# LesleyLai/cuda-path-tracer

Measured on AMD Instinct MI355X. Metric: Mrays/s at 1920×1080, 8 bounces, higher is better.
Workload: dtype f32

## Files before the change

cuda-path-tracer_amd/csrc/pt_bvh_gpu.hip:

```cpp
#include <hip/hip_runtime.h>

#include <algorithm>
#include <vector>

#include "../../include/ptcore.h"
#include "pt_bvh_rules.hpp"
#include "pt_device.hpp"
#include "pt_layout_rules.hpp"

namespace pt {
using namespace bvh_rules;
namespace {

constexpr uint32_t kFinished = 0xffffffffu;
constexpr uint32_t kBinWords = kBuckets * 7u;
constexpr uint32_t kSerialNode = 32u;

__device__ __forceinline__ uint32_t enc(float f)
{
  const uint32_t b = __float_as_uint(f);
  return (b & 0x80000000u) ? ~b : (b | 0x80000000u);
}
__device__ __forceinline__ float dec(uint32_t e) { return __uint_as_float((e & 0x80000000u) ? (e & 0x7fffffffu) : ~e); }

// ... 695 lines not shown
  layout_rules::quantise_node(q, nk, lo, hi, refs);
  uint4* out = reinterpret_cast<uint4*>(w.nodes_q) + 4u * (size_t)w.wbegin[x];
  for (int j = 0; j < 4; ++j) out[j] = make_uint4(q[4 * j], q[4 * j + 1], q[4 * j + 2], q[4 * j + 3]);
}

__global__ __launch_bounds__(256) void k_lay_instance_tris(m4 m, const float* positions, const uint32_t* indices,
                                                           const uint32_t* tri_order, uint32_t T, float4* out)
{
  const uint32_t k = blockIdx.x * 256u + threadIdx.x;
  if (k >= T) return;
  const uint32_t* idx = indices + 3u * (size_t)tri_order[k];
  const float* q0 = positions + 3u * (size_t)idx[0];
  const float* q1 = positions + 3u * (size_t)idx[1];
  const float* q2 = positions + 3u * (size_t)idx[2];
  layout_rules::instance_triangle(m, mk3(q0[0], q0[1], q0[2]), mk3(q1[0], q1[1], q1[2]), mk3(q2[0], q2[1], q2[2]), out + kTriVec4 * (size_t)k);
}

}

int build_layouts_device(hipStream_t stream, const float4* d_bvh, uint32_t count, const std::vector<uint32_t>& level_base,
                         DeviceLayouts* out)
{
  *out = DeviceLayouts{};
  if (count == 0u) return PTC_OK;
  if (level_base.size() < 2u || level_base.front() != 0u || level_base.back() != count) return PTC_ERR_INVALID;
  const uint32_t T = (count + 1u) / 2u;
  const size_t N = count;
  Pool pool;
  LayoutWork w{};
  w.tree.bvh = d_bvh;
// ... 59 lines not shown
  out->dummy_ref = w.dummy_ref;
  out->root_min[0] = root[0].x; out->root_min[1] = root[0].y; out->root_min[2] = root[0].z;
  out->root_max[0] = root[1].x; out->root_max[1] = root[1].y; out->root_max[2] = root[1].z;
  outputs.allocs.clear();
  return PTC_OK;
}

void launch_instance_triangles(hipStream_t stream, const m4& m, const float* d_positions, const uint32_t* d_indices,
                               const uint32_t* d_tri_order, uint32_t triangles, float4* d_out)
{
  if (triangles == 0u) return;
  hipLaunchKernelGGL(k_lay_instance_tris, dim3((triangles + 255u) / 256u), dim3(256), 0, stream, m, d_positions, d_indices,
                     d_tri_order, triangles, d_out);
}

}
```

cuda-path-tracer_amd/csrc/pt_device.hpp:

```cpp
#pragma once

#include <hip/hip_runtime.h>
#include <stdint.h>

#include <vector>

#include "../../include/ptcore.h"
#include "pt_math.hpp"

namespace pt {

constexpr int kWave = 64;
constexpr int kChunk = 64;
constexpr int kStackDepth = 64;
constexpr int kMaxBounces = 64;
constexpr int kWorkSlots = 4;
#ifndef PT_T4_LDS
#define PT_T4_LDS 24
#endif
constexpr int kLds4 = PT_T4_LDS;
static_assert(kLds4 >= 4 && kLds4 <= kStackDepth, "PT_T4_LDS out of range");

constexpr uint32_t kFlagStackOverflow = 1u;
constexpr uint32_t kFlagDispatchOrder = 2u;
// ... 17 lines not shown

#ifndef PT_TRI_VEC4
#define PT_TRI_VEC4 4
#endif
constexpr uint32_t kTriVec4 = PT_TRI_VEC4;
constexpr uint32_t kLeafBit = 0x80000000u;
constexpr uint32_t kNoChild = 0xffffffffu;

struct DMeshView {
  const float* positions;
  const uint32_t* indices;
  const float4* bvh;
  const float4* wide;
  const float4* leaf_parent;
  const uint4* bvh4q;
  uint32_t bvh4_root;
  uint32_t dummy_ref;
  float root_min[3];
  float root_max[3];
  uint32_t root_ref;
  uint32_t bvh_node_count;
};

struct DBand {
  uint32_t pix_begin, width, rank, nranks, block_rows;
};
PT_HD uint32_t band_pixel(const DBand& b, uint32_t s)
{
  if (b.nranks <= 1u) return b.pix_begin + s;
  const uint32_t lr = s / b.width, x = s - lr * b.width;
// ... 16 lines not shown
  uint32_t width;
  DBand band;
  uint8_t beam_of[32];
};
constexpr uint32_t kSphereTab = 8u;
struct DScene {
  const DObject* objects;
  const uint32_t* object_material;
  const float4* spheres;
  const DMaterial* materials;
  DMeshView cur;
  const DMeshView* mesh_views;
  const uint32_t* object_mesh;
  const float4* tris;
  const uint32_t* object_tri_base;
  uint32_t* slow_stack;
  uint2* spill;
  uint32_t spill_stride;
  uint32_t spill_cap;
  uint32_t lds_cap;
  uint32_t force_slow;
  uint32_t static_eighths;
  uint32_t refill_lanes;
  uint32_t split_idle;
  uint32_t object_count;
  const float4* sphere_ball;
  uint32_t lanes_run;
  uint32_t fold_run;
  DBeam beam;
};
// ... 104 lines not shown
                     std::vector<uint32_t>* level_base);

struct DeviceLayouts {
  uint32_t* nodes_q = nullptr;
  float4* leaf_parent = nullptr;
  uint32_t* tri_order = nullptr;
  float4* wide = nullptr;
  uint32_t wide4_nodes = 0, wide4_depth = 0, triangles = 0, inner_nodes = 0;
  uint32_t root_ref4 = 0, root_ref2 = 0, dummy_ref = 0;
  float root_min[3] = {0, 0, 0}, root_max[3] = {0, 0, 0};
};
int build_layouts_device(hipStream_t stream, const float4* d_bvh, uint32_t count, const std::vector<uint32_t>& level_base,
                         DeviceLayouts* out);
void launch_instance_triangles(hipStream_t stream, const m4& m, const float* d_positions, const uint32_t* d_indices,
                               const uint32_t* d_tri_order, uint32_t triangles, float4* d_out);

void launch_raygen(hipStream_t s, const DCameras& cams, const DBatchInfo& bi, DBand band, uint32_t pix_count,
                   DPaths paths, DeviceCounters* counters, const DObject* objects = nullptr, uint32_t filt_begin = 0u,
                   uint32_t filt_end = 0u, uint32_t* worklist = nullptr, DHits hits = DHits{nullptr, nullptr},
                   unsigned long long* tile_desc = nullptr, uint32_t tile_stride = 0u, uint32_t epoch = 0u,
                   bool finish_misses = false, DFrame fb = DFrame{nullptr, nullptr}, bool staged = false);
void launch_trace(hipStream_t s, const DScene& scene, DPaths paths, DHits hits, uint32_t max_paths, int bounce,
                  DeviceCounters* counters, bool count_tests, int variant);
void launch_spheres(hipStream_t s, const DScene& scene, uint32_t obj_begin, uint32_t obj_end, bool first, DPaths paths, DHits hits,
                    uint32_t max_paths, int bounce, DeviceCounters* counters, const DBatchInfo& bi, uint32_t filt_begin = 0u,
                    uint32_t filt_end = 0u, uint32_t* worklist = nullptr, unsigned long long* tile_desc = nullptr,
                    uint32_t tile_stride = 0u, uint32_t epoch = 0u);
void launch_traverse_run(hipStream_t s, const DScene& scene, uint32_t obj_begin, uint32_t obj_end, bool first, DPaths paths,
                         DHits hits, int bounce, int work_slot, DeviceCounters* counters, bool count_tests, uint32_t waves,
                         uint32_t* slow_list, const uint32_t* order, const DBatchInfo& bi, bool listed = false);
// ... 55 lines not shown
```

cuda-path-tracer_amd/csrc/pt_kernels.hip:

```cpp




#include "pt_device.hpp"
#include "pt_rng.hpp"
#include "pt_beam_rules.hpp"
#include "pt_feed_rules.hpp"
static_assert(pt::beam_rules::kLeaf == pt::kLeafBit, "pt_beam_rules.hpp restates the leaf bit of the four-wide node (pt_device.hpp)");
static_assert((uint32_t)pt::beam_rules::kEntries == pt::kBeamEntries, "pt_beam_rules.hpp restates the entries per tile (pt_device.hpp)");
static_assert(pt::feed_rules::kBatch == (uint32_t)pt::kWave, "a feed batch is one wavefront's worth of rays");
#include <float.h>

namespace pt {

#include "pt_kernels_common.inc"

template <bool kCount>
__global__ __launch_bounds__(kWave) void k_trace(DScene sc, DPaths paths, DHits hits, int bounce, DeviceCounters* counters)
{
  __shared__ uint32_t s_stack[kStackDepth * kWave];
  const uint32_t n = counters->live[bounce];
  const uint32_t s = blockIdx.x * kWave + threadIdx.x;
  if (blockIdx.x * kWave >= n) return;
  bool hit = false;
// ... 74 lines not shown
  generate_ray(cam, x0, y1, o, d01);
  generate_ray(cam, x1, y1, o, d11);
  generate_ray(cam, 0.5f * (x0 + x1), 0.5f * (y0 + y1), o, dc);
  const beam_rules::Frustum fr = beam_rules::make_frustum(xform_point(obj->inv_m, o), xform_vector(obj->inv_m, d00), xform_vector(obj->inv_m, d10),
                                                          xform_vector(obj->inv_m, d01), xform_vector(obj->inv_m, d11), xform_vector(obj->inv_m, dc));
  f3 lo4[4], hi4[4];
  uint32_t ref4[4];
  int n = 0;
  if (sc.cur.bvh_node_count != 0u)
    n = beam_rules::tile_entries(reinterpret_cast<const uint32_t*>(sc.cur.bvh4q), node_count4, sc.cur.bvh4_root, ld3(sc.cur.root_min), ld3(sc.cur.root_max), fr,
                                 lo4, hi4, ref4);
  float4* e = out + (size_t)id * (2u * kBeamEntries);
#pragma unroll
  for (int k = 0; k < (int)kBeamEntries; ++k) {
    if (k < n) {
      e[2 * k] = make_float4(lo4[k].x, lo4[k].y, lo4[k].z, __uint_as_float(ref4[k]));
      e[2 * k + 1] = make_float4(hi4[k].x, hi4[k].y, hi4[k].z, 0.0f);
    } else {
      e[2 * k] = make_float4(__builtin_inff(), __builtin_inff(), __builtin_inff(), __uint_as_float(kNoChild));
      e[2 * k + 1] = make_float4(-__builtin_inff(), -__builtin_inff(), -__builtin_inff(), 0.0f);
    }
  }
}

template <bool kCount, bool kFirst, bool kBeam = false>
__global__ __launch_bounds__(kWave) __attribute__((amdgpu_waves_per_eu(PT_T4_WAVES, PT_T4_WAVES)))
void k_traverse4(DScene sc, uint32_t obj_index, DPaths paths, DHits hits, int bounce, int work_slot,
                 DeviceCounters* counters, uint32_t* slow_list, const uint32_t* order, DBatchInfo bi, int listed)
{
  traverse4_walk<kCount, kFirst, kBeam>(sc, obj_index, paths, hits, bounce, work_slot, counters, slow_list, order, bi, listed != 0);
  uint32_t prev = 0u;
// ... 150 lines not shown
```

cuda-path-tracer_amd/csrc/pt_layout_rules.hpp:

```cpp
#pragma once

#include <cmath>

#include "pt_math.hpp"

namespace pt {
namespace layout_rules {

PT_HD void collapse_costs(float area_x, const float* bl, const float* br, float* b)
{
  float node_cost = bl[0] + br[2];
  node_cost = sel_min(node_cost, bl[1] + br[1]);
  node_cost = sel_min(node_cost, bl[2] + br[0]);
  b[0] = area_x + node_cost;
  b[1] = sel_min(b[0], bl[0] + br[0]);
  b[2] = sel_min(b[1], sel_min(bl[0] + br[1], bl[1] + br[0]));
  b[3] = sel_min(b[2], node_cost);
}

template <class Tree>
PT_HD int choose_children(const Tree& tree, const float* best, uint32_t x, uint32_t kids[4])
{
  int nk = 0;
  uint32_t stack_x[4];
// ... 63 lines not shown
        q[4 + a] = lo_q;
        q[7 + a] = hi_q;
        break;
      }
      ++e;
    }
    q[a] = __builtin_bit_cast(uint32_t, origin);
    exps |= (uint32_t)(e + 127) << (8 * a);
  }
  q[3] = (exps & 0xffu) << 23;
  q[10] = ((exps >> 8) & 0xffu) << 23;
  q[11] = ((exps >> 16) & 0xffu) << 23;
  for (int k = 0; k < 4; ++k) q[12 + k] = refs[k];
}

PT_HD void instance_triangle(const m4& m, f3 q0, f3 q1, f3 q2, float4* out)
{
  const f3 p0 = xform_point(m, q0), p1 = xform_point(m, q1), p2 = xform_point(m, q2);
  const f3 e1 = p1 - p0;
  const f3 e2 = p2 - p0;
  const f3 n = normalize(cross(e1, e2));
  out[0] = make_float4(p0.x, p0.y, p0.z, e1.x);
  out[1] = make_float4(e1.y, e1.z, e2.x, e2.y);
  out[2] = make_float4(e2.z, n.x, n.y, n.z);
}

}
}
```

cuda-path-tracer_amd/csrc/pt_walk.inc:

```
struct BatchFeed {
  DeviceCounters* ctr;
  uint32_t stride, count, bounce, work_slot, static_eighths, dyn_batch;
  bool listed;
  __device__ __forceinline__ uint32_t rays_of(uint32_t f) const { return listed ? ctr[f].list_count : ctr[f].live[bounce]; }
  uint32_t home_f, home_r, home_base, home_rs, stat_next, stat_step, stat_count;
  bool in_static, done;

  static __device__ __forceinline__ uint32_t region_size_of(uint32_t n) { return feed_rules::region_size_of(n); }
  static __device__ __forceinline__ uint32_t region_len_of(uint32_t n, uint32_t rs, uint32_t r) { return feed_rules::region_len_of(n, rs, r); }
  static __device__ __forceinline__ uint32_t pos_of(uint32_t rs, uint32_t r, uint32_t local) { return feed_rules::pos_of(rs, r, local); }
  __device__ __forceinline__ uint32_t static_batches_of(uint32_t len) const
  {
    return feed_rules::static_batches_of(len, static_eighths);
  }
  __device__ __forceinline__ void init(DeviceCounters* ctr_, const DBatchInfo& bi, int bounce_, int work_slot_,
                                       uint32_t static_eighths_, bool listed_ = false)
  {
    ctr = ctr_;
    listed = listed_;
    stride = bi.stride;
    count = bi.count;
    bounce = (uint32_t)bounce_;
    work_slot = (uint32_t)work_slot_;
    static_eighths = gridDim.x >= 8u * count ? static_eighths_ : 0u;
// ... 283 lines not shown
  __shared__ unsigned long long s_grp_best[kWave];
  __shared__ uint32_t s_grp_count[kWave];
  __shared__ uint32_t s_leader[kWave];
  __shared__ uint32_t s_pair[kWave];
  typedef __attribute__((address_space(3))) uint32_t lds_u32;
  lds_u32* stack = (lds_u32*)s_stack + threadIdx.x;
  const uint32_t gid = blockIdx.x * kWave + threadIdx.x;
  uint32_t n_max = 0u;
  if (!kPersist) {
    for (uint32_t f = 0; f < bi.count; ++f) n_max = max(n_max, listed ? counters[f].list_count : counters[f].live[bounce]);
    if (n_max == 0u) return 0;
  }
  const DObject* obj = sc.objects + obj_index;
  const uint32_t mat = sc.object_material[obj_index];
  const float4* tris = sc.tris + kTriVec4 * (size_t)sc.object_tri_base[obj_index];
  if (!kPersist && blockIdx.x >= ((n_max + kWave - 1u) / kWave + 8u) * bi.count) return 0;
  auto uni = [](float v) { return __uint_as_float((uint32_t)__builtin_amdgcn_readfirstlane((int)__float_as_uint(v))); };
  const f3 obj_bmin = mk3(uni(obj->bmin[0]), uni(obj->bmin[1]), uni(obj->bmin[2]));
  const f3 obj_bmax = mk3(uni(obj->bmax[0]), uni(obj->bmax[1]), uni(obj->bmax[2]));
#ifdef PT_TAILPROF
  const unsigned long long tp_start = wall_clock64();
  unsigned long long tp_exhausted = 0ull;
  uint32_t tp_iters = 0u, tp_splits = 0u, tp_iters_exh = 0u, tp_lanes_exh = 0u;
  unsigned long long tp_c_split = 0ull, tp_c_retire = 0ull, tp_c_step = 0ull, tp_lanes_tail = 0ull;
#endif
  BatchFeed feed;
  PersistFeed pfeed;
  if (kPersist) {
    pfeed.init(pa->st, counters, bi, blockIdx.x);
    if (threadIdx.x < (uint32_t)kMaxBatch) s_pend[threadIdx.x] = 0u;
// ... 166 lines not shown
      limit = d_limit;
      slot = d_slot;
      cur = ((lds_u32*)s_stack)[d_sbase * kWave + (int)d];
      sp = sbase = 0;
      ray_boxes = 0u;
      const uint32_t leader = s_leader[d];
      s_leader[threadIdx.x] = leader;
      __hip_atomic_fetch_add(&s_grp_count[leader], 1u, __ATOMIC_RELAXED, __HIP_MEMORY_SCOPE_WORKGROUP);
      active = true;
    }
    if (can_give && drank < pairs) ++sbase;
  };

  auto step = [&]() {
    if (active) {
      const bool is_leaf = (cur & kLeafBit) != 0u;
      const uint32_t index = cur & ~kLeafBit;
      typedef uint32_t u32x4 __attribute__((ext_vector_type(4)));
      u32x4 w0, w1, w2, w3;
      constexpr bool kLeaf48 = kTriVec4 == 3u;
      const char* rec = is_leaf ? reinterpret_cast<const char*>(tris) + (16u * kTriVec4) * (size_t)index
                                : reinterpret_cast<const char*>(sc.cur.bvh4q) + 64u * (size_t)index;
      const char* rec3 = rec + (kLeaf48 && is_leaf ? 32 : 48);
      const int top = sp - 1;
      const uint32_t below_addr = (uint32_t)(uintptr_t)(stack + min(max(top, 0), lds_cap - 1) * kWave);
      uint32_t below;
      asm volatile(
          "global_load_dwordx4 %0, %5, off\n\t"
          "global_load_dwordx4 %1, %5, off offset:16\n\t"
          "global_load_dwordx4 %2, %5, off offset:32\n\t"
          "global_load_dwordx4 %3, %6, off\n\t"
          "ds_read_b32 %4, %7\n\t"
          "s_waitcnt vmcnt(0) lgkmcnt(0)"
          : "=&v"(w0), "=&v"(w1), "=&v"(w2), "=&v"(w3), "=&v"(below)
          : "v"(rec), "v"(rec3), "v"(below_addr)
          : "memory");
      if (__builtin_expect(top >= lds_cap, 0)) below = sc.spill[(size_t)(top - lds_cap) * sc.spill_stride + gid].x;
      below = top >= sbase ? below : kNoChild;
      const uint4 q0 = make_uint4(w0.x, w0.y, w0.z, w0.w), q1 = make_uint4(w1.x, w1.y, w1.z, w1.w);
      const uint4 q2 = make_uint4(w2.x, w2.y, w2.z, w2.w), q3 = make_uint4(w3.x, w3.y, w3.z, w3.w);
      if (!is_leaf) {
        if (kCount) ++tally.nodes;
        const f3 org = mk3(__uint_as_float(q0.x), __uint_as_float(q0.y), __uint_as_float(q0.z));
        const f3 ax = mk3(__uint_as_float(q0.w) * inv.x, __uint_as_float(q2.z) * inv.y, __uint_as_float(q2.w) * inv.z);
        const f3 bn = mk3(__builtin_fmaf(org.x, inv.x, oin.x), __builtin_fmaf(org.y, inv.y, oin.y), __builtin_fmaf(org.z, inv.z, oin.z));
        const f3 bf = mk3(__builtin_fmaf(org.x, inv.x, oif.x), __builtin_fmaf(org.y, inv.y, oif.y), __builtin_fmaf(org.z, inv.z, oif.z));
        const uint32_t nqx = neg_x ? q1.w : q1.x, fqx = neg_x ? q1.x : q1.w;
        const uint32_t nqy = neg_y ? q2.x : q1.y, fqy = neg_y ? q1.y : q2.x;
        const uint32_t nqz = neg_z ? q2.y : q1.z, fqz = neg_z ? q1.z : q2.y;
        float key[4];
        uint32_t ref[4] = {q3.x, q3.y, q3.z, q3.w};
#pragma unroll
        for (int c = 0; c < 4; ++c) {
          const float cnx = (float)((nqx >> (8 * c)) & 0xffu), cny = (float)((nqy >> (8 * c)) & 0xffu), cnz = (float)((nqz >> (8 * c)) & 0xffu);
          const float cfx = (float)((fqx >> (8 * c)) & 0xffu), cfy = (float)((fqy >> (8 * c)) & 0xffu), cfz = (float)((fqz >> (8 * c)) & 0xffu);
          const float tn = fmaxf(fmaxf(fmaxf(__builtin_fmaf(cnx, ax.x, bn.x), __builtin_fmaf(cny, ax.y, bn.y)),
                                       __builtin_fmaf(cnz, ax.z, bn.z)), 0.0f);
          const float tf = fminf(fminf(fminf(__builtin_fmaf(cfx, ax.x, bf.x), __builtin_fmaf(cfy, ax.y, bf.y)),
                                       __builtin_fmaf(cfz, ax.z, bf.z)), limit);
          if (kCount && ref[c] != sc.cur.dummy_ref) { ++tally.boxes; ++ray_boxes; }
          key[c] = tn <= tf ? tn : __builtin_inff();
        }
        auto cx = [&](int a, int b) {
          const bool sw = key[b] < key[a];
          const float ka = sw ? key[b] : key[a], kb = sw ? key[a] : key[b];
          const uint32_t ra = sw ? ref[b] : ref[a], rb = sw ? ref[a] : ref[b];
          key[a] = ka;
          key[b] = kb;
          ref[a] = ra;
          ref[b] = rb;
        };
        cx(0, 1);
        cx(2, 3);
        cx(0, 2);
        cx(1, 3);
// ... 8 lines not shown
          stack[sp * kWave] = ref[1];
          sp += key[1] < __builtin_inff() ? 1 : 0;
        } else {
          if (key[3] < __builtin_inff()) push(ref[3]);
          if (key[2] < __builtin_inff()) push(ref[2]);
          if (key[1] < __builtin_inff()) push(ref[1]);
        }
        if (key[0] < __builtin_inff()) {
          cur = ref[0];
        } else {
          cur = below;
          sp = max(sp - 1, sbase);
        }
      } else {
        if (kCount) ++tally.tris;
        const f3 p0 = mk3(__uint_as_float(q0.x), __uint_as_float(q0.y), __uint_as_float(q0.z));
        const f3 e1 = mk3(__uint_as_float(q0.w), __uint_as_float(q1.x), __uint_as_float(q1.y));
        const f3 e2 = mk3(__uint_as_float(q1.z), __uint_as_float(q1.w), __uint_as_float(q2.x));
#if PT_FLAT_TRI
        const f3 h = cross(rd, e2);
        const float a = dot(e1, h);
        const f3 sv = ro - p0;
        const float f = 1.0f / a;
        const float u = f * dot(sv, h);
        const f3 qv = cross(sv, e1);
        const float w = f * dot(rd, qv);
        const float t = f * dot(e2, qv);
        const bool hit = !(a > -0.0000001f && a < 0.0000001f) & !(u < 0.0f || u > 1.0f) & !(w < 0.0f || u + w > 1.0f) &
                         !(t < tmin) & (t < best_t || (t == best_t && (int)index > best_k));
        best_t = hit ? t : best_t;
// ... 105 lines not shown
          if (__builtin_expect(!(finite_f(inv.x) && finite_f(inv.y) && finite_f(inv.z) && finite_f(tol.x + tol.y + tol.z)) ||
                               sc.force_slow == 1u, 0)) {
            if (kPersist) set_aside(counters + cur_frame, pa->slow_list + (size_t)cur_frame * bi.stride, slot & kSlotMask);
            else set_aside(counters, slow_list, slot);
            wrote = true;
            go = false;
          } else {
            oin = oi - tol;
            oif = oi + tol;
            neg_x = inv.x < 0.0f;
            neg_y = inv.y < 0.0f;
            neg_z = inv.z < 0.0f;
            best_t = t_in;
            best_k = -1;
            limit = scale * best_t * 1.001f;
            cur = sc.cur.bvh4_root;
            sp = sbase = 0;
            ray_boxes = 0u;
            if (kBeam) {
              float key[4];
              uint32_t ref[4];
#pragma unroll
              for (int c = 0; c < 4; ++c) {
                const float4 lo = eb[2 * c], hi = eb[2 * c + 1];
                const float tn = fmaxf(fmaxf(fmaxf(__builtin_fmaf(neg_x ? hi.x : lo.x, inv.x, oin.x), __builtin_fmaf(neg_y ? hi.y : lo.y, inv.y, oin.y)),
                                             __builtin_fmaf(neg_z ? hi.z : lo.z, inv.z, oin.z)), 0.0f);
                const float tf = fminf(fminf(fminf(__builtin_fmaf(neg_x ? lo.x : hi.x, inv.x, oif.x), __builtin_fmaf(neg_y ? lo.y : hi.y, inv.y, oif.y)),
                                             __builtin_fmaf(neg_z ? lo.z : hi.z, inv.z, oif.z)), limit);
                key[c] = tn <= tf ? tn : __builtin_inff();
                ref[c] = __float_as_uint(lo.w);
                if (kCount && key[c] < __builtin_inff()) { ++tally.boxes; ++ray_boxes; }
// ... 133 lines not shown
```

cuda-path-tracer_amd/csrc/ptcore_checks.cpp:

```cpp
#include "ptcore_ctx.hpp"

using namespace pt;
using namespace ptcd;

extern "C" {

int ptc_check_beam(const float* positions, uint32_t vertex_count, const uint32_t* indices, uint32_t index_count, const float* object_m16,
                   const ptc_camera* camera, uint32_t width, uint32_t height, uint32_t stride, uint64_t* stats5, float* entries_out)
{
  if (!positions || !indices || !camera || index_count == 0u || index_count % 3u || width < 2u || height < 2u || stride == 0u) return PTC_ERR_INVALID;
  std::vector<ptc_bvh_node> nodes((size_t)index_count / 3u * 2u);
  uint32_t depth = 0;
  const int rc = build_bvh(positions, vertex_count, indices, index_count, nodes.data(), &depth);
  if (rc < 0) return rc;
  WideAccel wide;
  if (int r = build_wide(nodes.data(), (uint32_t)rc, wide)) return r;
  Wide4Accel w4;
  if (int r = build_wide4(nodes.data(), (uint32_t)rc, w4)) return r;
  m4 m{};
  for (int c = 0; c < 4; ++c)
    for (int r = 0; r < 4; ++r) m.c[c][r] = object_m16 ? object_m16[4 * c + r] : (c == r ? 1.0f : 0.0f);
  const m4 inv_m = inverse(m);
  const DCamera cam = make_camera(*camera, width, height);
  auto gen = [&](float fx, float fy, f3& o, f3& d) {
// ... 51 lines not shown
      }
      if (ref >= n4) return HitRec{true, 0xffffffffu, -1.0f};
      const uint32_t* q = nq + 16u * (size_t)ref;
      for (int c = 0; c < 4; ++c) {
        f3 lo, hi;
        if (!beam_rules::child_box(q, c, lo, hi)) continue;
        if (slab(lo, hi, o, inv, best.t)) stack.push_back(q[12 + c]);
      }
    }
    return best;
  };
  uint64_t tiles = 0, empty = 0, entries = 0, rays = 0, hits = 0;
  int bad = 0;
  const uint32_t tiles_x = (width + kBeamTile - 1u) / kBeamTile, tiles_y = (height + kBeamTile - 1u) / kBeamTile;
  const uint32_t root_ref4[1] = {w4.root_ref};
  for (uint32_t ty = 0; ty < tiles_y; ++ty)
    for (uint32_t tx = 0; tx < tiles_x; ++tx) {
      const float x0 = (float)(tx * kBeamTile) - 0.05f, x1 = (float)((tx + 1u) * kBeamTile) + 0.05f;
      const float y0 = (float)(ty * kBeamTile) - 0.05f, y1 = (float)((ty + 1u) * kBeamTile) + 0.05f;
      f3 o, d00, d10, d01, d11, dc;
      gen(x0, y0, o, d00);
      gen(x1, y0, o, d10);
      gen(x0, y1, o, d01);
      gen(x1, y1, o, d11);
      gen(0.5f * (x0 + x1), 0.5f * (y0 + y1), o, dc);
      const beam_rules::Frustum fr = beam_rules::make_frustum(xform_point(inv_m, o), xform_vector(inv_m, d00), xform_vector(inv_m, d10),
                                                              xform_vector(inv_m, d01), xform_vector(inv_m, d11), xform_vector(inv_m, dc));
      f3 lo4[4], hi4[4];
      uint32_t ref4[4];
      const int n = beam_rules::tile_entries(nq, n4, w4.root_ref, root_lo, root_hi, fr, lo4, hi4, ref4);
      if (entries_out) {
        float* e = entries_out + ((size_t)ty * tiles_x + tx) * 32u;
        for (int k = 0; k < 4; ++k) {
          const float inf = __builtin_inff();
          uint32_t ref = k < n ? ref4[k] : kNoChild;
          float refbits;
          std::memcpy(&refbits, &ref, 4);
          const float rec[8] = {k < n ? lo4[k].x : inf, k < n ? lo4[k].y : inf, k < n ? lo4[k].z : inf, refbits,
                                k < n ? hi4[k].x : -inf, k < n ? hi4[k].y : -inf, k < n ? hi4[k].z : -inf, 0.0f};
          std::memcpy(e + 8 * k, rec, sizeof rec);
        }
      }
      ++tiles;
      empty += n == 0;
      entries += (uint64_t)n;
      for (int k = 0; k < n; ++k)
        if (!(ref4[k] & kLeafBit) && ref4[k] >= n4) ++bad;
      for (uint32_t py = ty * kBeamTile; py < std::min(height, (ty + 1u) * kBeamTile); py += stride)
        for (uint32_t px = tx * kBeamTile; px < std::min(width, (tx + 1u) * kBeamTile); px += stride) {
          const float jit[5][2] = {{0.0f, 0.0f}, {1.0f, 0.0f}, {0.0f, 1.0f}, {1.0f, 1.0f}, {0.5f, 0.5f}};
// ... 240 lines not shown
```

cuda-path-tracer_amd/csrc/ptcore_ctx.hpp:

```cpp
#pragma once

#include "../../include/ptcore.h"

#include <hip/hip_runtime.h>

#include <algorithm>
#include <chrono>
#include <cmath>
#include <cstddef>
#include <cstdio>
#include <cstdlib>
#include <cstring>
#include <new>
#include <string>
#include <unordered_map>
#include <vector>

#include "pt_device.hpp"
#include "pt_host.hpp"
#include "pt_beam_rules.hpp"
#include "pt_feed_rules.hpp"

using namespace pt;

// ... 130 lines not shown
  bool sphere_lanes = true;
  bool sphere_fold = true;
  bool beam = true;
  int persist = 0;
  uint32_t persist_service_every = 5;
  uint32_t persist_help_tiles = 8;
  uint32_t persist_min_frames = 2;
  uint64_t scene_serial = 0;
  uint32_t beam_tiles_x = 0, beam_tiles_y = 0;
  uint32_t traverse_waves = 5120;
  uint32_t refill_lanes = 32;
  uint32_t static_eighths = 4;
  bool merge_instances = true;
  bool bvh_on_device = true;
  bool layout_on_device = true;
  uint64_t layout_counts[5] = {0, 0, 0, 0, 0};
  uint32_t split_idle = 8;
  uint32_t min_waves = 1024;
  uint32_t small_waves = 3072;
  uint32_t small_rays_per_lane = 4;
  uint32_t run_waves = 3072;
  uint32_t est_live[2 * (kMaxBounces + 1)] = {};
  bool est_valid = false;
  bool filter_rays = true;
  bool prefold = true;
  bool fused_shade = true;
  int ray_sort = 0;
  int denoise_variant = 0;
  uint32_t lds_entries = kLds4;
  int force_slow = 0;

// ... 66 lines not shown
```

cuda-path-tracer_amd/csrc/ptcore_scene.cpp:

```cpp
#include "ptcore_ctx.hpp"

using namespace pt;
using namespace ptcd;

namespace {

static void sphere_ball_of(const ptc_object& o, const ptc_sphere* spheres, uint32_t sphere_count, uint32_t material, float4* out)
{
  out[0] = make_float4(0.f, 0.f, 0.f, -1.0f);
  for (uint32_t k = 1; k < kSphereTab; ++k) out[k] = make_float4(0.f, 0.f, 0.f, 0.f);
  if (o.type != 0u || o.index >= sphere_count) return;
  const float* m = o.m;
  if (!(m[3] == 0.0f && m[7] == 0.0f && m[11] == 0.0f && m[15] == 1.0f)) return;
  const ptc_sphere& sp = spheres[o.index];
  double a[3][3];
  for (int r = 0; r < 3; ++r)
    for (int c = 0; c < 3; ++c) a[r][c] = (double)m[4 * c + r];
  double g[3][3];
  double frob2 = 0.0;
  for (int i = 0; i < 3; ++i)
    for (int j = 0; j < 3; ++j) {
      g[i][j] = 0.0;
      for (int k = 0; k < 3; ++k) g[i][j] += a[k][i] * a[k][j];
      frob2 += a[i][j] * a[i][j];
// ... 389 lines not shown
      m4 m;
      std::memcpy(&m, s->objects[i].m, sizeof m);
      float4* dst = tris + (size_t)tri_base[i] * kTriVec4;
      if (w.tri_order_dev) {
        launch_instance_triangles(ctx->stream, m, w.view.positions, w.view.indices, w.tri_order_dev, w.triangles, dst);
      } else {
        host_tris.assign((size_t)w.triangles * kTriVec4, make_float4(0.f, 0.f, 0.f, 0.f));
        build_instance_triangles(m, w.positions, w.indices, w.tri_order_host, host_tris.data());
        HIP_TRY(ctx, hipMemcpyAsync(dst, host_tris.data(), host_tris.size() * sizeof(float4), hipMemcpyHostToDevice, ctx->stream));
        HIP_TRY(ctx, hipStreamSynchronize(ctx->stream));
      }
    }
    HIP_TRY(ctx, hipStreamSynchronize(ctx->stream));
    d.tris = tris;
    if (int rc = upload(ctx, ctx->scene_allocs, &d.object_tri_base, tri_base.data(), tri_base.size())) return rc;
    lap(times.triangles_ms);
  }
  ctx->mesh_views.clear();
  ctx->mesh_nodes4.clear();
  for (const MeshWork& w : meshes) {
    ctx->mesh_views.push_back(w.view);
    ctx->mesh_nodes4.push_back(w.w4_nodes);
  }
  ctx->object_mesh = object_mesh;
  if (int rc = upload(ctx, ctx->scene_allocs, &d.mesh_views, ctx->mesh_views.data(), ctx->mesh_views.size())) return rc;
  if (int rc = upload(ctx, ctx->scene_allocs, &d.object_mesh, object_mesh.data(), object_mesh.size())) return rc;
  if (!ctx->mesh_views.empty()) d.cur = ctx->mesh_views[0];
  lap(times.copy_ms);

  {
// ... 53 lines not shown
  times.total_ms = std::chrono::duration<float, std::milli>(std::chrono::steady_clock::now() - t_start).count();
  ctx->upload_times = times;
  return PTC_OK;
}

int ptc_build_bvh_device(ptc_ctx* ctx, const float* positions, uint32_t vertex_count, const uint32_t* indices,
                         uint32_t index_count, ptc_bvh_node* nodes, uint32_t* max_depth)
{
  if (!ctx || !positions || !indices || !nodes || index_count % 3u != 0u) return fail(ctx, PTC_ERR_INVALID, "bad arguments");
  if (int rc = bind_device(ctx)) return rc;
  return bvh_on_device(ctx, positions, vertex_count, indices, index_count, nodes, max_depth, nullptr);
}

int ptc_download_layout(ptc_ctx* ctx, int which, void* host, uint64_t capacity, uint64_t* bytes)
{
  if (!ctx || which < 0 || which > 4) return fail(ctx, PTC_ERR_INVALID, "layout: 0 bvh4q, 1 leaf_parent, 2 tris, 3 wide, 4 bvh");
  if (!ctx->has_scene) return fail(ctx, PTC_ERR_NO_SCENE, "no scene uploaded");
  if (int rc = bind_device(ctx)) return rc;
  const void* src[5] = {ctx->scene.cur.bvh4q, ctx->scene.cur.leaf_parent, ctx->scene.tris, ctx->scene.cur.wide, ctx->scene.cur.bvh};
  const uint64_t n = ctx->layout_counts[which];
  if (bytes) *bytes = n;
  if (!host) return PTC_OK;
  if (capacity < n) return fail(ctx, PTC_ERR_INVALID, "buffer too small");
  if (n) HIP_TRY(ctx, hipMemcpy(host, src[which], n, hipMemcpyDeviceToHost));
  return PTC_OK;
}

int ptc_get_upload_times(const ptc_ctx* ctx, ptc_upload_times* out)
{
  if (!ctx || !out) return PTC_ERR_INVALID;
  *out = ctx->upload_times;
  return PTC_OK;
}

// ... 16 lines not shown
```

cuda-path-tracer_amd/path_tracer.py:

```python
import ctypes as C
from dataclasses import dataclass
from enum import IntEnum

import numpy as np

from . import _capi
from .scene_description import Camera, FlatScene, SceneDescription


class GPUMethod(IntEnum):
    megakernel = 0
    streaming = 1


class DisplayBufferType(IntEnum):
    final = 0
    color = 1
    normal = 2
    depth = 3


@dataclass
class EdgeAvoidingATrousDenoiser:
    filter_size: int = 10
# ... 191 lines not shown
        t = mesh.triangle_count()
        nodes = np.zeros(max(2 * t - 1, 1), dtype=BVH_NODE_DTYPE)
        depth = C.c_uint32(0)
        rc = self._lib.ptc_build_bvh_device(self._ctx, mesh.positions.ctypes.data_as(C.POINTER(C.c_float)), len(mesh.positions),
                                            mesh.indices.ctypes.data_as(C.POINTER(C.c_uint32)), len(mesh.indices),
                                            nodes.ctypes.data_as(C.POINTER(_capi.ptc_bvh_node)), C.byref(depth))
        if rc < 0:
            self._check(rc)
        return nodes[:rc], depth.value

    def upload_times(self):
        t = _capi.ptc_upload_times()
        self._check(self._lib.ptc_get_upload_times(self._ctx, C.byref(t)))
        return {k: (int(getattr(t, k)) if k.endswith("on_device") else round(float(getattr(t, k)), 2)) for k, _ in t._fields_}

    LAYOUTS = {"bvh4q": 0, "leaf_parent": 1, "tris": 2, "wide": 3, "bvh": 4}

    def download_layout(self, which):
        n = C.c_uint64(0)
        self._check(self._lib.ptc_download_layout(self._ctx, self.LAYOUTS[which], None, 0, C.byref(n)))
        out = np.zeros(n.value, dtype=np.uint8)
        self._check(self._lib.ptc_download_layout(self._ctx, self.LAYOUTS[which], out.ctypes.data, n.value, None))
        return out

    def set_trace_variant(self, variant):
        self._check(self._lib.ptc_set_trace_variant(self._ctx, int(variant)))

    def set_param(self, name, value):
        self._check(self._lib.ptc_set_param(self._ctx, name.encode(), int(value)))

    def set_profiling(self, time_trace_kernel=False, count_tests=False):
# ... 41 lines not shown
```

Before: 7113.

## Store BVH4 traversal as unified 48-byte walk records with implicit child indices

Builds a per-object walk array where each BVH4 node's children sit in four consecutive 64-byte records, each holding either the quantised child node or the leaf triangle inline. Child references are packed into spare exponent-free bits, so a traversal step issues three 16-byte loads from one address instead of four loads from two (node vs triangle) buffers, and the leaf/inner branch is resolved from the loaded data. Beam entries are remapped to walk indices through a walk_of table. This costs extra memory, since triangles are duplicated and dummy slots are padded, plus a build kernel at scene upload.

```diff
diff --git a/cuda-path-tracer_amd/csrc/pt_bvh_gpu.hip b/cuda-path-tracer_amd/csrc/pt_bvh_gpu.hip
--- a/cuda-path-tracer_amd/csrc/pt_bvh_gpu.hip
+++ b/cuda-path-tracer_amd/csrc/pt_bvh_gpu.hip
@@ -733,6 +733,18 @@
   const float* q1 = positions + 3u * (size_t)idx[1];
   const float* q2 = positions + 3u * (size_t)idx[2];
   layout_rules::instance_triangle(m, mk3(q0[0], q0[1], q0[2]), mk3(q1[0], q1[1], q1[2]), mk3(q2[0], q2[1], q2[2]), out + kTriVec4 * (size_t)k);
+}
+
+__global__ __launch_bounds__(256) void k_lay_walk(const uint32_t* nodes_q, uint32_t n4, uint32_t root_ref4, uint32_t dummy_ref,
+                                                  const float4* tris, uint4* out, uint32_t* walk_of)
+{
+  const uint32_t w = blockIdx.x * 256u + threadIdx.x;
+  if (w >= 4u * (n4 + 1u)) return;
+  const uint32_t ref = layout_rules::walk_slot_ref(nodes_q, root_ref4, dummy_ref, w);
+  uint32_t r[16];
+  layout_rules::walk_record(nodes_q, dummy_ref, reinterpret_cast<const uint32_t*>(tris), 4u * kTriVec4, ref, r);
+  for (int j = 0; j < 4; ++j) out[4u * (size_t)w + j] = make_uint4(r[4 * j], r[4 * j + 1], r[4 * j + 2], r[4 * j + 3]);
+  if (walk_of) layout_rules::walk_index_of(nodes_q, n4, root_ref4, dummy_ref, w, walk_of);
 }
 
 }
@@ -822,4 +834,12 @@
                      d_tri_order, triangles, d_out);
 }
 
-}
+void launch_walk_records(hipStream_t stream, const uint32_t* d_nodes_q, uint32_t n4, uint32_t root_ref4, uint32_t dummy_ref,
+                         const float4* d_tris, uint4* d_out, uint32_t* d_walk_of)
+{
+  const uint32_t records = 4u * (n4 + 1u);
+  hipLaunchKernelGGL(k_lay_walk, dim3((records + 255u) / 256u), dim3(256), 0, stream, d_nodes_q, n4, root_ref4, dummy_ref, d_tris,
+                     d_out, d_walk_of);
+}
+
+}
diff --git a/cuda-path-tracer_amd/csrc/pt_device.hpp b/cuda-path-tracer_amd/csrc/pt_device.hpp
--- a/cuda-path-tracer_amd/csrc/pt_device.hpp
+++ b/cuda-path-tracer_amd/csrc/pt_device.hpp
@@ -6,6 +6,7 @@
 #include <vector>
 
 #include "../../include/ptcore.h"
+#include "pt_layout_rules.hpp"
 #include "pt_math.hpp"
 
 namespace pt {
@@ -55,6 +56,7 @@
   const float4* wide;
   const float4* leaf_parent;
   const uint4* bvh4q;
+  const uint32_t* walk_of;
   uint32_t bvh4_root;
   uint32_t dummy_ref;
   float root_min[3];
@@ -101,6 +103,8 @@
   const uint32_t* object_mesh;
   const float4* tris;
   const uint32_t* object_tri_base;
+  const uint4* walk;
+  const uint32_t* object_walk_base;
   uint32_t* slow_stack;
   uint2* spill;
   uint32_t spill_stride;
@@ -235,6 +239,8 @@
                          DeviceLayouts* out);
 void launch_instance_triangles(hipStream_t stream, const m4& m, const float* d_positions, const uint32_t* d_indices,
                                const uint32_t* d_tri_order, uint32_t triangles, float4* d_out);
+void launch_walk_records(hipStream_t stream, const uint32_t* d_nodes_q, uint32_t n4, uint32_t root_ref4, uint32_t dummy_ref,
+                         const float4* d_tris, uint4* d_out, uint32_t* d_walk_of);
 
 void launch_raygen(hipStream_t s, const DCameras& cams, const DBatchInfo& bi, DBand band, uint32_t pix_count,
                    DPaths paths, DeviceCounters* counters, const DObject* objects = nullptr, uint32_t filt_begin = 0u,
diff --git a/cuda-path-tracer_amd/csrc/pt_kernels.hip b/cuda-path-tracer_amd/csrc/pt_kernels.hip
--- a/cuda-path-tracer_amd/csrc/pt_kernels.hip
+++ b/cuda-path-tracer_amd/csrc/pt_kernels.hip
@@ -112,7 +112,8 @@
 #pragma unroll
   for (int k = 0; k < (int)kBeamEntries; ++k) {
     if (k < n) {
-      e[2 * k] = make_float4(lo4[k].x, lo4[k].y, lo4[k].z, __uint_as_float(ref4[k]));
+      const uint32_t w = sc.cur.walk_of[(ref4[k] & kLeafBit) ? node_count4 + (ref4[k] & ~kLeafBit) : ref4[k]];
+      e[2 * k] = make_float4(lo4[k].x, lo4[k].y, lo4[k].z, __uint_as_float(w));
       e[2 * k + 1] = make_float4(hi4[k].x, hi4[k].y, hi4[k].z, 0.0f);
     } else {
       e[2 * k] = make_float4(__builtin_inff(), __builtin_inff(), __builtin_inff(), __uint_as_float(kNoChild));
diff --git a/cuda-path-tracer_amd/csrc/pt_layout_rules.hpp b/cuda-path-tracer_amd/csrc/pt_layout_rules.hpp
--- a/cuda-path-tracer_amd/csrc/pt_layout_rules.hpp
+++ b/cuda-path-tracer_amd/csrc/pt_layout_rules.hpp
@@ -101,6 +101,47 @@
   for (int k = 0; k < 4; ++k) q[12 + k] = refs[k];
 }
 
+constexpr uint32_t kWalkStepMask = 0x7f800000u;
+constexpr uint32_t kWalkLeafTag = 0x80000000u;
+
+PT_HD uint32_t walk_slot_ref(const uint32_t* nodes_q, uint32_t root_ref4, uint32_t dummy_ref, uint32_t w)
+{
+  const uint32_t b = w >> 2, c = w & 3u;
+  if (b == 0u) return c == 0u ? root_ref4 : dummy_ref;
+  return nodes_q[16u * (size_t)(b - 1u) + 12u + c];
+}
+
+PT_HD void walk_record(const uint32_t* nodes_q, uint32_t dummy_ref, const uint32_t* tris, uint32_t tri_words, uint32_t ref, uint32_t out[16])
+{
+  for (int k = 0; k < 16; ++k) out[k] = 0u;
+  if (ref & 0x80000000u) {
+    const uint32_t r = ref & 0x7fffffffu;
+    const uint32_t* t = tris + tri_words * (size_t)r;
+    for (int k = 0; k < 9; ++k) out[k] = t[k];
+    out[9] = r;
+    out[11] = kWalkLeafTag;
+    return;
+  }
+  const uint32_t* q = nodes_q + 16u * (size_t)ref;
+  const uint32_t first = 4u * (ref + 1u);
+  uint32_t nk = 0u;
+  for (int c = 0; c < 4; ++c) nk += q[12 + c] != dummy_ref ? 1u : 0u;
+  for (int k = 0; k < 12; ++k) out[k] = q[k];
+  out[3] |= first & 0x7fffffu;
+  out[10] |= first >> 23;
+  out[11] |= nk;
+}
+
+PT_HD void walk_index_of(const uint32_t* nodes_q, uint32_t n4, uint32_t root_ref4, uint32_t dummy_ref, uint32_t w, uint32_t* walk_of)
+{
+  const uint32_t ref = walk_slot_ref(nodes_q, root_ref4, dummy_ref, w);
+  if (ref == dummy_ref) {
+    if (w == 1u) walk_of[n4 + (dummy_ref & 0x7fffffffu)] = 1u;
+    return;
+  }
+  walk_of[(ref & 0x80000000u) ? n4 + (ref & 0x7fffffffu) : ref] = w;
+}
+
 PT_HD void instance_triangle(const m4& m, f3 q0, f3 q1, f3 q2, float4* out)
 {
   const f3 p0 = xform_point(m, q0), p1 = xform_point(m, q1), p2 = xform_point(m, q2);
diff --git a/cuda-path-tracer_amd/csrc/pt_walk.inc b/cuda-path-tracer_amd/csrc/pt_walk.inc
--- a/cuda-path-tracer_amd/csrc/pt_walk.inc
+++ b/cuda-path-tracer_amd/csrc/pt_walk.inc
@@ -321,6 +321,7 @@
   const DObject* obj = sc.objects + obj_index;
   const uint32_t mat = sc.object_material[obj_index];
   const float4* tris = sc.tris + kTriVec4 * (size_t)sc.object_tri_base[obj_index];
+  const uint4* walk = sc.walk + 4u * (size_t)sc.object_walk_base[obj_index];
   if (!kPersist && blockIdx.x >= ((n_max + kWave - 1u) / kWave + 8u) * bi.count) return 0;
   auto uni = [](float v) { return __uint_as_float((uint32_t)__builtin_amdgcn_readfirstlane((int)__float_as_uint(v))); };
   const f3 obj_bmin = mk3(uni(obj->bmin[0]), uni(obj->bmin[1]), uni(obj->bmin[2]));
@@ -517,42 +518,39 @@
 
   auto step = [&]() {
     if (active) {
-      const bool is_leaf = (cur & kLeafBit) != 0u;
-      const uint32_t index = cur & ~kLeafBit;
       typedef uint32_t u32x4 __attribute__((ext_vector_type(4)));
-      u32x4 w0, w1, w2, w3;
-      constexpr bool kLeaf48 = kTriVec4 == 3u;
-      const char* rec = is_leaf ? reinterpret_cast<const char*>(tris) + (16u * kTriVec4) * (size_t)index
-                                : reinterpret_cast<const char*>(sc.cur.bvh4q) + 64u * (size_t)index;
-      const char* rec3 = rec + (kLeaf48 && is_leaf ? 32 : 48);
+      u32x4 w0, w1, w2;
+      const char* rec = reinterpret_cast<const char*>(walk) + 64u * (size_t)cur;
       const int top = sp - 1;
       const uint32_t below_addr = (uint32_t)(uintptr_t)(stack + min(max(top, 0), lds_cap - 1) * kWave);
       uint32_t below;
       asm volatile(
-          "global_load_dwordx4 %0, %5, off\n\t"
-          "global_load_dwordx4 %1, %5, off offset:16\n\t"
-          "global_load_dwordx4 %2, %5, off offset:32\n\t"
-          "global_load_dwordx4 %3, %6, off\n\t"
-          "ds_read_b32 %4, %7\n\t"
+          "global_load_dwordx4 %0, %4, off\n\t"
+          "global_load_dwordx4 %1, %4, off offset:16\n\t"
+          "global_load_dwordx4 %2, %4, off offset:32\n\t"
+          "ds_read_b32 %3, %5\n\t"
           "s_waitcnt vmcnt(0) lgkmcnt(0)"
-          : "=&v"(w0), "=&v"(w1), "=&v"(w2), "=&v"(w3), "=&v"(below)
-          : "v"(rec), "v"(rec3), "v"(below_addr)
+          : "=&v"(w0), "=&v"(w1), "=&v"(w2), "=&v"(below)
+          : "v"(rec), "v"(below_addr)
           : "memory");
       if (__builtin_expect(top >= lds_cap, 0)) below = sc.spill[(size_t)(top - lds_cap) * sc.spill_stride + gid].x;
       below = top >= sbase ? below : kNoChild;
       const uint4 q0 = make_uint4(w0.x, w0.y, w0.z, w0.w), q1 = make_uint4(w1.x, w1.y, w1.z, w1.w);
-      const uint4 q2 = make_uint4(w2.x, w2.y, w2.z, w2.w), q3 = make_uint4(w3.x, w3.y, w3.z, w3.w);
+      const uint4 q2 = make_uint4(w2.x, w2.y, w2.z, w2.w);
+      const bool is_leaf = (int)q2.w < 0;
       if (!is_leaf) {
         if (kCount) ++tally.nodes;
         const f3 org = mk3(__uint_as_float(q0.x), __uint_as_float(q0.y), __uint_as_float(q0.z));
-        const f3 ax = mk3(__uint_as_float(q0.w) * inv.x, __uint_as_float(q2.z) * inv.y, __uint_as_float(q2.w) * inv.z);
+        const f3 ax = mk3(__uint_as_float(q0.w & layout_rules::kWalkStepMask) * inv.x, __uint_as_float(q2.z & layout_rules::kWalkStepMask) * inv.y,
+                          __uint_as_float(q2.w & layout_rules::kWalkStepMask) * inv.z);
+        const uint32_t first = (q0.w & 0x7fffffu) | (q2.z << 23);
         const f3 bn = mk3(__builtin_fmaf(org.x, inv.x, oin.x), __builtin_fmaf(org.y, inv.y, oin.y), __builtin_fmaf(org.z, inv.z, oin.z));
         const f3 bf = mk3(__builtin_fmaf(org.x, inv.x, oif.x), __builtin_fmaf(org.y, inv.y, oif.y), __builtin_fmaf(org.z, inv.z, oif.z));
         const uint32_t nqx = neg_x ? q1.w : q1.x, fqx = neg_x ? q1.x : q1.w;
         const uint32_t nqy = neg_y ? q2.x : q1.y, fqy = neg_y ? q1.y : q2.x;
         const uint32_t nqz = neg_z ? q2.y : q1.z, fqz = neg_z ? q1.z : q2.y;
         float key[4];
-        uint32_t ref[4] = {q3.x, q3.y, q3.z, q3.w};
+        uint32_t ref[4] = {first, first | 1u, first | 2u, first | 3u};
 #pragma unroll
         for (int c = 0; c < 4; ++c) {
           const float cnx = (float)((nqx >> (8 * c)) & 0xffu), cny = (float)((nqy >> (8 * c)) & 0xffu), cnz = (float)((nqz >> (8 * c)) & 0xffu);
@@ -561,7 +559,7 @@
                                        __builtin_fmaf(cnz, ax.z, bn.z)), 0.0f);
           const float tf = fminf(fminf(fminf(__builtin_fmaf(cfx, ax.x, bf.x), __builtin_fmaf(cfy, ax.y, bf.y)),
                                        __builtin_fmaf(cfz, ax.z, bf.z)), limit);
-          if (kCount && ref[c] != sc.cur.dummy_ref) { ++tally.boxes; ++ray_boxes; }
+          if (kCount && (uint32_t)c < (q2.w & 7u)) { ++tally.boxes; ++ray_boxes; }
           key[c] = tn <= tf ? tn : __builtin_inff();
         }
         auto cx = [&](int a, int b) {
@@ -600,6 +598,7 @@
         }
       } else {
         if (kCount) ++tally.tris;
+        const uint32_t index = q2.y;
         const f3 p0 = mk3(__uint_as_float(q0.x), __uint_as_float(q0.y), __uint_as_float(q0.z));
         const f3 e1 = mk3(__uint_as_float(q0.w), __uint_as_float(q1.x), __uint_as_float(q1.y));
         const f3 e2 = mk3(__uint_as_float(q1.z), __uint_as_float(q1.w), __uint_as_float(q2.x));
@@ -735,7 +734,7 @@
             best_t = t_in;
             best_k = -1;
             limit = scale * best_t * 1.001f;
-            cur = sc.cur.bvh4_root;
+            cur = 0u;
             sp = sbase = 0;
             ray_boxes = 0u;
             if (kBeam) {
diff --git a/cuda-path-tracer_amd/csrc/ptcore_checks.cpp b/cuda-path-tracer_amd/csrc/ptcore_checks.cpp
--- a/cuda-path-tracer_amd/csrc/ptcore_checks.cpp
+++ b/cuda-path-tracer_amd/csrc/ptcore_checks.cpp
@@ -89,6 +89,8 @@
   int bad = 0;
   const uint32_t tiles_x = (width + kBeamTile - 1u) / kBeamTile, tiles_y = (height + kBeamTile - 1u) / kBeamTile;
   const uint32_t root_ref4[1] = {w4.root_ref};
+  std::vector<uint32_t> walk_of((size_t)n4 + index_count / 3u + 1u, 0u);
+  for (uint32_t w = 0; w < 4u * (n4 + 1u); ++w) layout_rules::walk_index_of(nq, n4, w4.root_ref, w4.dummy_ref, w, walk_of.data());
   for (uint32_t ty = 0; ty < tiles_y; ++ty)
     for (uint32_t tx = 0; tx < tiles_x; ++tx) {
       const float x0 = (float)(tx * kBeamTile) - 0.05f, x1 = (float)((tx + 1u) * kBeamTile) + 0.05f;
@@ -108,7 +110,7 @@
         float* e = entries_out + ((size_t)ty * tiles_x + tx) * 32u;
         for (int k = 0; k < 4; ++k) {
           const float inf = __builtin_inff();
-          uint32_t ref = k < n ? ref4[k] : kNoChild;
+          uint32_t ref = k < n ? walk_of[(ref4[k] & kLeafBit) ? n4 + (ref4[k] & ~kLeafBit) : ref4[k]] : kNoChild;
           float refbits;
           std::memcpy(&refbits, &ref, 4);
           const float rec[8] = {k < n ? lo4[k].x : inf, k < n ? lo4[k].y : inf, k < n ? lo4[k].z : inf, refbits,
diff --git a/cuda-path-tracer_amd/csrc/ptcore_ctx.hpp b/cuda-path-tracer_amd/csrc/ptcore_ctx.hpp
--- a/cuda-path-tracer_amd/csrc/ptcore_ctx.hpp
+++ b/cuda-path-tracer_amd/csrc/ptcore_ctx.hpp
@@ -168,7 +168,7 @@
   bool merge_instances = true;
   bool bvh_on_device = true;
   bool layout_on_device = true;
-  uint64_t layout_counts[5] = {0, 0, 0, 0, 0};
+  uint64_t layout_counts[6] = {0, 0, 0, 0, 0, 0};
   uint32_t split_idle = 8;
   uint32_t min_waves = 1024;
   uint32_t small_waves = 3072;
diff --git a/cuda-path-tracer_amd/csrc/ptcore_scene.cpp b/cuda-path-tracer_amd/csrc/ptcore_scene.cpp
--- a/cuda-path-tracer_amd/csrc/ptcore_scene.cpp
+++ b/cuda-path-tracer_amd/csrc/ptcore_scene.cpp
@@ -427,6 +427,35 @@
     HIP_TRY(ctx, hipStreamSynchronize(ctx->stream));
     d.tris = tris;
     if (int rc = upload(ctx, ctx->scene_allocs, &d.object_tri_base, tri_base.data(), tri_base.size())) return rc;
+    std::vector<uint32_t> walk_base(s->object_count, 0u);
+    size_t walk_records = 0;
+    for (uint32_t i = 0; i < s->object_count; ++i) {
+      if (s->objects[i].type != 1u || object_mesh[i] >= mesh_count || meshes[object_mesh[i]].triangles == 0u) continue;
+      walk_base[i] = (uint32_t)walk_records;
+      walk_records += 4u * ((size_t)meshes[object_mesh[i]].w4_nodes + 1u);
+      if (walk_records > 0xffffffffull) return fail(ctx, PTC_ERR_OOM, "too many walk records");
+    }
+    uint4* walk = nullptr;
+    if (int rc = dev_alloc(ctx, ctx->scene_allocs, &walk, walk_records * 4u)) return rc;
+    std::vector<bool> mapped(mesh_count, false);
+    for (uint32_t i = 0; i < s->object_count; ++i) {
+      if (s->objects[i].type != 1u || object_mesh[i] >= mesh_count) continue;
+      MeshWork& w = meshes[object_mesh[i]];
+      if (w.triangles == 0u) continue;
+      uint32_t* walk_of = nullptr;
+      if (!mapped[object_mesh[i]]) {
+        if (int rc = dev_alloc(ctx, ctx->scene_allocs, &walk_of, (size_t)w.w4_nodes + w.triangles + 1u)) return rc;
+        w.view.walk_of = walk_of;
+        mapped[object_mesh[i]] = true;
+      }
+      launch_walk_records(ctx->stream, reinterpret_cast<const uint32_t*>(w.view.bvh4q), w.w4_nodes, w.view.bvh4_root, w.view.dummy_ref,
+                          tris + (size_t)tri_base[i] * kTriVec4, walk + 4u * (size_t)walk_base[i], walk_of);
+      HIP_TRY(ctx, hipGetLastError());
+    }
+    HIP_TRY(ctx, hipStreamSynchronize(ctx->stream));
+    d.walk = walk;
+    if (int rc = upload(ctx, ctx->scene_allocs, &d.object_walk_base, walk_base.data(), walk_base.size())) return rc;
+    ctx->layout_counts[5] = (uint64_t)walk_records * 64u;
     lap(times.triangles_ms);
   }
   ctx->mesh_views.clear();
@@ -510,10 +539,11 @@
 
 int ptc_download_layout(ptc_ctx* ctx, int which, void* host, uint64_t capacity, uint64_t* bytes)
 {
-  if (!ctx || which < 0 || which > 4) return fail(ctx, PTC_ERR_INVALID, "layout: 0 bvh4q, 1 leaf_parent, 2 tris, 3 wide, 4 bvh");
+  if (!ctx || which < 0 || which > 5) return fail(ctx, PTC_ERR_INVALID, "layout: 0 bvh4q, 1 leaf_parent, 2 tris, 3 wide, 4 bvh, 5 walk");
   if (!ctx->has_scene) return fail(ctx, PTC_ERR_NO_SCENE, "no scene uploaded");
   if (int rc = bind_device(ctx)) return rc;
-  const void* src[5] = {ctx->scene.cur.bvh4q, ctx->scene.cur.leaf_parent, ctx->scene.tris, ctx->scene.cur.wide, ctx->scene.cur.bvh};
+  const void* src[6] = {ctx->scene.cur.bvh4q, ctx->scene.cur.leaf_parent, ctx->scene.tris, ctx->scene.cur.wide, ctx->scene.cur.bvh,
+                        ctx->scene.walk};
   const uint64_t n = ctx->layout_counts[which];
   if (bytes) *bytes = n;
   if (!host) return PTC_OK;
diff --git a/cuda-path-tracer_amd/path_tracer.py b/cuda-path-tracer_amd/path_tracer.py
--- a/cuda-path-tracer_amd/path_tracer.py
+++ b/cuda-path-tracer_amd/path_tracer.py
@@ -229,7 +229,7 @@
         self._check(self._lib.ptc_get_upload_times(self._ctx, C.byref(t)))
         return {k: (int(getattr(t, k)) if k.endswith("on_device") else round(float(getattr(t, k)), 2)) for k, _ in t._fields_}
 
-    LAYOUTS = {"bvh4q": 0, "leaf_parent": 1, "tris": 2, "wide": 3, "bvh": 4}
+    LAYOUTS = {"bvh4q": 0, "leaf_parent": 1, "tris": 2, "wide": 3, "bvh": 4, "walk": 5}
 
     def download_layout(self, which):
         n = C.c_uint64(0)
```

New measurement: 7269 (median of 6 runs). 2.2% higher.
